# arhix52/Strelka

Measured on AMD Instinct MI355X. Metric: Mray/s, higher is better.
Workload: dtype f32; 1 GPU; kitchen stand-in (SURVEY 8d C3): 1724134 unique triangles, 2022 instances of 153 meshes, 4 rect + 1 distant light, 60/25/10/5 % diffuse/glossy/metal/glass; resolution=1920x1080, bounces=4, spp=64, tile=32, world_size=1, parallelism=single GPU, rays_per_frame=839862650

## Files before the change

strelka_amd/csrc/skh_kernels.h:

```cpp
#pragma once
#include "skh_bvh.h"
#include "skh_env.h"
#include "skh_emit.h"
#include "skh_blend.h"

namespace skh
{

struct DevInstance
{
    float w2o[12];
    int rootRef;
    uint32_t mask;
    uint32_t type;
    uint32_t pad;
};
struct HostInstance
{
    float o2w[12];
    uint32_t type, geom, material, light;
};

#define SKH_WORLD_CURVES 2
#define SKH_SEG_STRIDE 8
// ... 444 lines not shown
        atomicAdd(&stats->rayTicksAfterDry[A], rayTicks);
        atomicAdd(&stats->waveTicksAfterDry[A], now - dryAt);
    }
#endif
    if (COUNT)
    {
        const uint32_t a = wave_sum(tc.nodes), b = wave_sum(tc.prims), c2 = wave_sum(tc.segs), d2 = wave_sum(tc.insts);
#ifdef SKH_LANE_PROFILE
        cy[5] = __builtin_readcyclecounter() - cyStart;
        if (lane == 0)
        {
            atomicAdd(&stats->cyc[ANY_HIT ? 1 : 0][6], cy[5]);
            atomicAdd(&stats->cyc[ANY_HIT ? 1 : 0][7], __builtin_amdgcn_s_memrealtime() - rtStart);
        }
        for (int k = 0; k < 7; ++k)
        {
            uint32_t hi = wave_max((uint32_t)(cy[k] >> 8));
            if (lane == 0)
                atomicAdd(&stats->cyc[ANY_HIT ? 1 : 0][k == 6 ? 8 : k], (unsigned long long)hi << 8);
        }
#endif
        if (lane == 0)
        {
            atomicAdd(&stats->nodes[ANY_HIT ? 1 : 0], (unsigned long long)a);
            atomicAdd(&stats->prims[ANY_HIT ? 1 : 0], (unsigned long long)b);
            atomicAdd(&stats->segs[ANY_HIT ? 1 : 0], (unsigned long long)c2);
            atomicAdd(&stats->insts[ANY_HIT ? 1 : 0], (unsigned long long)d2);
#ifdef SKH_LANE_PROFILE
            for (int k = 0; k < 10; ++k)
                atomicAdd(&stats->wave[ANY_HIT ? 1 : 0][k], (unsigned long long)wv[k]);
#endif
        }
    }
#undef SKH_LP
}

__global__ void k_hair_consts(const Material* __restrict__ mats, uint32_t n, HairConst* __restrict__ out)
{
    const uint32_t i = blockIdx.x * blockDim.x + threadIdx.x;
    if (i < n)
        out[i] = hair_const(mats[i]);
}

SKH_DI bool slot_to_pixel(const FrameP& fp, const uint32_t* __restrict__ tileXY, uint32_t slot, uint32_t& px, uint32_t& py)
{
    const uint32_t tile = slot >> (2 * fp.tileShift);
    const uint32_t m = slot & ((1u << (2 * fp.tileShift)) - 1u);
    px = tileXY[2 * tile] + compact1by1(m);
    py = tileXY[2 * tile + 1] + compact1by1(m >> 1);
    return px < fp.width && py < fp.height;
}

#define SKH_COMPACT_MAX_WAVES 8
SKH_DI uint32_t block_compact(bool emit, uint32_t* counter, uint32_t* s_wave )
{
    const uint32_t lane = threadIdx.x & 63u, wave = threadIdx.x >> 6, nw = blockDim.x >> 6;
    const unsigned long long m = __ballot(emit);
    if (lane == 0)
        s_wave[wave] = (uint32_t)__popcll(m);
    __syncthreads();
    if (threadIdx.x == 0)
    {
        uint32_t tot = 0;
        for (uint32_t w = 0; w < nw; ++w)
        {
            const uint32_t cnt = s_wave[w];
            s_wave[w] = tot;
            tot += cnt;
        }
        s_wave[SKH_COMPACT_MAX_WAVES] = tot ? atomicAdd(counter, tot) : 0u;
    }
    __syncthreads();
    const uint32_t r = s_wave[SKH_COMPACT_MAX_WAVES] + s_wave[wave] + rank_below(m);
    __syncthreads();
    return r;
}
SKH_DI void block_compact2(bool emitA, uint32_t* counterA, bool emitB, uint32_t* counterB, uint32_t* s_wave2, uint32_t& ia, uint32_t& ib)
{
    const uint32_t lane = threadIdx.x & 63u, wave = threadIdx.x >> 6, nw = blockDim.x >> 6;
    const unsigned long long ma = __ballot(emitA), mb = __ballot(emitB);
    uint32_t* sa = s_wave2;
    uint32_t* sb = s_wave2 + SKH_COMPACT_MAX_WAVES + 1;
    if (lane == 0)
    {
        sa[wave] = (uint32_t)__popcll(ma);
        sb[wave] = (uint32_t)__popcll(mb);
    }
    __syncthreads();
    if (threadIdx.x == 0 || threadIdx.x == 64)
    {
        uint32_t* sw = threadIdx.x == 0 ? sa : sb;
        uint32_t tot = 0;
        for (uint32_t w = 0; w < nw; ++w)
        {
            const uint32_t cnt = sw[w];
            sw[w] = tot;
            tot += cnt;
        }
        sw[SKH_COMPACT_MAX_WAVES] = tot ? atomicAdd(threadIdx.x == 0 ? counterA : counterB, tot) : 0u;
    }
    if (nw == 1 && threadIdx.x == 0)
    {
        uint32_t tot = sb[0];
        sb[0] = 0;
        sb[SKH_COMPACT_MAX_WAVES] = tot ? atomicAdd(counterB, tot) : 0u;
    }
    __syncthreads();
    ia = sa[SKH_COMPACT_MAX_WAVES] + sa[wave] + rank_below(ma);
    ib = sb[SKH_COMPACT_MAX_WAVES] + sb[wave] + rank_below(mb);
}

__global__ void __launch_bounds__(512) k_raygen(FrameP fp, const uint32_t* __restrict__ tileXY, uint32_t sampleOffset, RayQ rq,
                                               uint32_t* __restrict__ counter, PathS ps, const uint32_t* __restrict__ qBase,
                                               const uint32_t* __restrict__ subStride, uint32_t blocksPerSub, uint32_t validPerSub,
                                               uint32_t launchCell, uint32_t perWave)
{
    __shared__ uint32_t s_wave[SKH_COMPACT_MAX_WAVES + 1];
    const uint32_t span = launchCell * fp.batch, lc = blockIdx.x / span, inSpan = blockIdx.x - lc * span;
    const uint32_t nb = min(launchCell, blocksPerSub - lc * launchCell);
    const uint32_t sub = inSpan / nb, bi = lc * launchCell + (inSpan - sub * nb);
    const uint32_t slot = bi * blockDim.x + threadIdx.x;
    const uint32_t path = sub * fp.numSlots + slot;
    uint32_t px = 0, py = 0;
    const bool active = sub < fp.batch && slot < fp.numSlots && slot_to_pixel(fp, tileXY, slot, px, py);
    v3 o = mk3(0.0f), d = mk3(0.0f);
    if (active)
    {
// ... 206 lines not shown
}
SKH_DI v3 emit_sample_texel(const MtexP& m, const DevScene& sc, uint32_t instance, uint32_t prim, float ux, float uy)
{
    const HostInstance* __restrict__ hi = sc.instances + instance;
    const uint32_t mid0 = hi->material == 0xffffffffu ? 0u : hi->material, mid = mid0 < sc.numMaterials ? mid0 : 0u;
    const MtexEntry e = mtex_entry(m, mid);
    if (!mtex_valid(e.emission_texture, sc.numTextures))
        return mk3(1.0f);
    const float4* __restrict__ tp = sc.shadeTris + 6 * (size_t)(hi->light + prim);
    const float4 t3 = tp[3], t4 = tp[4];
    float u0, v0, u1, v1, u2, v2;
    unpack_uv(__float_as_uint(t3.w), u0, v0);
    unpack_uv(__float_as_uint(t4.x), u1, v1);
    unpack_uv(__float_as_uint(t4.y), u2, v2);
    const float su = sqrtf(ux);
    const float b0 = 1.0f - su, b1 = su * (1.0f - uy), b2 = su * uy;
    return mtex_emission_texel(tex_lookup_rgba8(sc.texels, sc.texDesc[e.emission_texture - 1u], (u0 * b0 + u1 * b1) + u2 * b2, (v0 * b0 + v1 * b1) + v2 * b2),
                               e.emission_channel);
}
__global__ void __launch_bounds__(256) k_material_probe(MtexP mt, const Material* __restrict__ materials, uint32_t numMaterials, const float4* __restrict__ Le,
                                                        const uint32_t* __restrict__ texels, const uint4* __restrict__ texDesc, uint32_t numTextures,
                                                        const uint32_t* __restrict__ material, const float* __restrict__ uv, uint32_t n, float* __restrict__ out)
{
    const uint32_t i = blockIdx.x * blockDim.x + threadIdx.x;
    if (i >= n)
        return;
    const uint32_t mid0 = material[i] == 0xffffffffu ? 0u : material[i], mid = mid0 < numMaterials ? mid0 : 0u;
    Material mat = materials[mid];
    const float4 l = Le[mid];
    v3 le = mk3(l.x, l.y, l.z);
    resolve_material(texels, texDesc, numTextures, mat, mtex_entry(mt, mid), le, uv[2 * (size_t)i], uv[2 * (size_t)i + 1]);
    float* o = out + 8 * (size_t)i;
    o[0] = mat.base_color[0], o[1] = mat.base_color[1], o[2] = mat.base_color[2], o[3] = mat.roughness, o[4] = mat.metallic;
    o[5] = le.x, o[6] = le.y, o[7] = le.z;
}
__global__ void __launch_bounds__(256) k_emit_probe_mtex(EmitP em, MtexP mt, DevScene sc, const float* __restrict__ in, uint32_t n, uint32_t* __restrict__ out)
{
    const uint32_t i = blockIdx.x * blockDim.x + threadIdx.x;
    if (i >= n)
        return;
    const float* q = in + 6 * (size_t)i;
    const EmitSample s = emit_sample(em, q[0], q[1], q[2], mk3(q[3], q[4], q[5]));
    const v3 Le = s.Le * emit_sample_texel(mt, sc, s.instance, s.prim, q[1], q[2]);
    uint32_t* o = out + 13 * (size_t)i;
    o[0] = __float_as_uint(s.point.x), o[1] = __float_as_uint(s.point.y), o[2] = __float_as_uint(s.point.z);
    o[3] = __float_as_uint(s.normal.x), o[4] = __float_as_uint(s.normal.y), o[5] = __float_as_uint(s.normal.z);
    o[6] = __float_as_uint(Le.x), o[7] = __float_as_uint(Le.y), o[8] = __float_as_uint(Le.z);
    o[9] = __float_as_uint(s.pdf), o[10] = __float_as_uint(s.dist), o[11] = s.instance, o[12] = s.prim;
}

#ifndef SKH_SHADE_WAVES
#define SKH_SHADE_WAVES(HAIR) ((HAIR) ? 4 : 5)
#endif
#define SKH_SHADE_ATTR(HAIR) __attribute__((amdgpu_waves_per_eu(SKH_SHADE_WAVES(HAIR), SKH_SHADE_WAVES(HAIR))))
#ifndef SKH_SHADE_BLOCK
#define SKH_SHADE_BLOCK 256
#endif
template <bool HAIR, bool ENV, bool EMIT, bool MTEX>
__global__ void __launch_bounds__(SKH_SHADE_BLOCK) SKH_SHADE_ATTR(HAIR)
    k_shade(DevScene sc, FrameP fp, uint32_t sampleOffset, uint32_t depth , const uint32_t* __restrict__ tileXY, RayQ rq,
            const uint32_t* __restrict__ countPtr, HitQ hq, PathS ps, RayQ nextQ, uint32_t* __restrict__ nextCount, RayQ shadowQ,
            float4* __restrict__ contrib, uint32_t* __restrict__ shadowCount, EnvP env, EmitP emit, MtexP mtex)
{
    constexpr bool LSHAPE = false;
    const LshapeP lsh = { nullptr };
#include "skh_shade_body.inc"
}
template <bool HAIR, bool ENV, bool EMIT, bool MTEX>
__global__ void __launch_bounds__(SKH_SHADE_BLOCK) SKH_SHADE_ATTR(HAIR)
    k_shade_lshape(DevScene sc, FrameP fp, uint32_t sampleOffset, uint32_t depth , const uint32_t* __restrict__ tileXY, RayQ rq,
                   const uint32_t* __restrict__ countPtr, HitQ hq, PathS ps, RayQ nextQ, uint32_t* __restrict__ nextCount, RayQ shadowQ,
                   float4* __restrict__ contrib, uint32_t* __restrict__ shadowCount, EnvP env, EmitP emit, MtexP mtex, LshapeP lsh)
{
    constexpr bool LSHAPE = true;
#include "skh_shade_body.inc"
}

__global__ void __launch_bounds__(256) k_lshape_probe(const Light* __restrict__ lights, uint32_t numLights, LshapeP lsh, uint32_t rectMethod, uint32_t kind,
                                                      const uint32_t* __restrict__ in, uint32_t n, float* __restrict__ out)
{
    const uint32_t i = blockIdx.x * blockDim.x + threadIdx.x;
    if (i >= n)
        return;
    const uint32_t* q = in + (kind == 0u ? 6u : 7u) * (size_t)i;
    const uint32_t lid = q[0];
    float* o = out + (kind == 0u ? 13u : 2u) * (size_t)i;
    if (lid >= numLights)
    {
        for (uint32_t k = 0; k < (kind == 0u ? 13u : 2u); ++k)
            o[k] = 0.0f;
        return;
    }
    const Light light = lights[lid];
    Lshape lse;
    lse.flags = 0u, lse.cosOuter = lse.cosInner = lse.focus = 0.0f, lse.axis = mk3(0.0f);
    if (lsh.table)
        lse = lshape_fetch(lsh, lid);
    const bool sampledDisc = light.type == 1 && (lse.flags & SKH_LSHAPE_SAMPLE_DISC) != 0u;
    if (kind == 0u)
    {
        const float ux = __uint_as_float(q[1]), uy = __uint_as_float(q[2]);
        const v3 P = mk3(__uint_as_float(q[3]), __uint_as_float(q[4]), __uint_as_float(q[5]));
        LightSample d;
        d.pointOnLight = mk3(0.0f), d.pdf = 0.0f, d.normal = mk3(0.0f), d.area = 0.0f, d.L = mk3(0.0f), d.distToLight = 0.0f;
        switch (light.type)
        {
        case 0:
            d = rectMethod == 0u ? sample_rect_light_uniform(light, ux, uy, P) : sample_rect_light(light, ux, uy, P);
            break;
        case 1:
            if (sampledDisc)
                d = sample_disc_light(light, ux, uy, P);
            break;
        case 2:
            d = sample_sphere_light(light, ux, uy, P);
            break;
        case 3:
            d = sample_distant_light(light, ux, uy);
            break;
        default:
            break;
        }
// ... 667 lines not shown
```

strelka_amd/csrc/skh_shade_body.inc:

```
    const uint32_t numPick = (ENV ? sc.numLights + (env.nee ? 1u : 0u) : sc.numLights) + (EMIT ? (emit.nee ? 1u : 0u) : 0u);
    __shared__ uint32_t s_wave[2 * (SKH_COMPACT_MAX_WAVES + 1)];
    __shared__ uint32_t s_sobol[SKH_SOBOL_LUT_WORDS];
#if SKH_MATERIALS_LDS
    __shared__ float4 s_mat[SKH_MATERIALS_LDS * 4];
#endif
    const uint32_t shard = blockIdx.x & (SKH_SHARDS - 1u), lb = blockIdx.x / SKH_SHARDS;
    const uint32_t n = countPtr[shard * SKH_COUNT_STRIDE];
    if (lb * blockDim.x >= n)
        return;
    const uint32_t il = lb * blockDim.x + threadIdx.x;
    const uint32_t i = shard * rq.region + il;
#ifdef SKH_LANE_PROFILE
    unsigned long long spc[8] = { 0, 0, 0, 0, 0, 0, 0, 0 }, spT = __builtin_readcyclecounter();
#define SKH_SP(k)                                                    \
    {                                                                \
        const unsigned long long t_ = __builtin_readcyclecounter();  \
        spc[k] += t_ - spT;                                          \
        spT = t_;                                                    \
    }
#else
#define SKH_SP(k)
#endif
    bool valid = il < n;
    uint32_t pid = 0;
    v3 rayO = mk3(0.0f), rayD = mk3(0.0f);
    float4 hr0 = make_float4(0.0f, 0.0f, 0.0f, 0.0f), hr1 = hr0;
    {
        constexpr int passes = ((SKH_SOBOL_LUT_WORDS / 4) + SKH_SHADE_BLOCK - 1) / SKH_SHADE_BLOCK;
        uint4 lut[passes];
#pragma unroll
        for (int k = 0; k < passes; ++k)
            if ((k + 1) * SKH_SHADE_BLOCK <= SKH_SOBOL_LUT_WORDS / 4 || threadIdx.x + k * SKH_SHADE_BLOCK < SKH_SOBOL_LUT_WORDS / 4)
                lut[k] = reinterpret_cast<const uint4*>(g_sobol_lut)[threadIdx.x + k * SKH_SHADE_BLOCK];
            else
                lut[k] = make_uint4(0u, 0u, 0u, 0u);
#if SKH_MATERIALS_LDS
        float4 mrow = make_float4(0.0f, 0.0f, 0.0f, 0.0f);
        static_assert(SKH_MATERIALS_LDS * 4 <= SKH_SHADE_BLOCK, "one float4 of the material table per thread");
        if (threadIdx.x < SKH_MATERIALS_LDS * 4 && threadIdx.x < sc.numMaterials * 4u)
            mrow = reinterpret_cast<const float4*>(sc.materials)[threadIdx.x];
#endif
#pragma unroll
        for (int k = 0; k < passes; ++k)
            if ((k + 1) * SKH_SHADE_BLOCK <= SKH_SOBOL_LUT_WORDS / 4 || threadIdx.x + k * SKH_SHADE_BLOCK < SKH_SOBOL_LUT_WORDS / 4)
                reinterpret_cast<uint4*>(s_sobol)[threadIdx.x + k * SKH_SHADE_BLOCK] = lut[k];
#if SKH_MATERIALS_LDS
        if (threadIdx.x < SKH_MATERIALS_LDS * 4)
            s_mat[threadIdx.x] = mrow;
#endif
    }
    __syncthreads();
    bool emitNext = false, emitShadow = false;
    v3 nextO = mk3(0.0f), nextD = mk3(0.0f), shO = mk3(0.0f), shD = mk3(0.0f), shC = mk3(0.0f);
    float shTmax = 0.0f;
    if (valid)
    {
        pid = rq.ids()[i];
        rayO = mk3(rq.plane(0)[i], rq.plane(1)[i], rq.plane(2)[i]);
        rayD = mk3(rq.plane(3)[i], rq.plane(4)[i], rq.plane(5)[i]);
        if (hq.primBits != 0u)
        {
            hr0 = *hq.rec16(i);
            const uint32_t w = __float_as_uint(hr0.w);
            hr1.x = __uint_as_float(w == 0xffffffffu ? w : w >> hq.primBits);
            hr1.y = __uint_as_float(w == 0xffffffffu ? w : ((w & ((1u << hq.primBits) - 1u)) | (hq.direct ? SKH_PRIM_DIRECT : 0u)));
        }
        else
            hr0 = hq.rec(i)[0], hr1 = hq.rec(i)[1];
        const float ht = hr0.x, hu = hr0.y, hv = hr0.z;
        const uint32_t hinst = __float_as_uint(hr1.x), hprim = __float_as_uint(hr1.y);
        float* P = ps.base;
        const size_t S = ps.stride;
        v3 throughput = depth == 0u ? mk3(1.0f) : mk3(P[pid], P[pid + S], P[pid + 2 * S]);
        v3 radiance = mk3(0.0f);
        bool radianceDirty = false;
#define SKH_RADIANCE_LOAD() radiance = mk3(ps.rad()[pid]), radianceDirty = true
        float lastBsdfPdf = depth == 0u ? 0.0f : P[pid + 6 * S];
        uint32_t flags = depth == 0u ? 0u : reinterpret_cast<uint32_t*>(P)[pid + 7 * S];
        bool inside = (flags & PF_INSIDE) != 0;
        bool specularBounce = (flags & PF_SPECULAR) != 0;
        uint32_t firstEvent = (flags >> PF_EVENT_SHIFT) & 3u;
        uint32_t px, py;
        const uint32_t sub = pid / fp.numSlots;
        slot_to_pixel(fp, tileXY, pid - sub * fp.numSlots, px, py);
        Sampler smp = init_sampler(px, py, fp.subframeIndex + sampleOffset + sub, fp.sppTotal, 52u);
        smp.depth = depth;
        uint32_t prdDepth = depth;
        v3 origin = rayO, dir = rayD;

        if (hinst == 0xffffffffu)
        {
            if constexpr (ENV)
            {
                const EnvEval ee = env_eval(env, rayD);
                SKH_RADIANCE_LOAD();
                if (depth == 0 || specularBounce || !env.nee)
                    radiance = radiance + throughput * ee.Le;
                else
                {
                    const float lightPdf = ee.pdf / (float)numPick;
                    const float misWeight = mis_weight_balance(lastBsdfPdf, lightPdf);
                    radiance = radiance + throughput * ee.Le * misWeight;
                }
            }
            else
            {
                const v3 bg = throughput * mk3(0.0f);
                if (!(bg.x == 0.0f && bg.y == 0.0f && bg.z == 0.0f))
                {
                    SKH_RADIANCE_LOAD();
                    radiance = radiance + bg;
                }
            }
            throughput = mk3(0.0f);
            prdDepth = fp.maxDepth;
        }
        else
        {
            SKH_SP(0)
            const HostInstance hi = sc.instances[hinst];
            const float* w2o = sc.inst[hinst].w2o;
            const bool directTv = (hprim & SKH_PRIM_DIRECT) != 0u;
            float4 tv[3], tx[2];
            const bool txWanted = HAIR || sc.numTextures != 0u;
            tx[0] = tx[1] = make_float4(0.0f, 0.0f, 0.0f, 0.0f);
            {
                const uint32_t recIdx = directTv ? (hprim & ~SKH_PRIM_DIRECT) : 0u;
                const float4* tp = sc.shadeTris + 6 * (size_t)(hq.primBits ? min(recIdx, hq.recClamp) : recIdx);
#pragma unroll
                for (int k = 0; k < 3; ++k)
                    tv[k] = tp[k];
                if (txWanted)
                    tx[0] = tp[3], tx[1] = tp[4];
            }
            asm volatile("" ::"v"(hi.type), "v"(hi.material), "v"(hi.light));
            if (hi.type == 1)
            {
                const uint32_t lidx = hi.light < sc.numLights ? hi.light : 0u;
                const Light& l = sc.lights[lidx];
                const v3 hitPoint = rayO + ht * rayD;
                if constexpr (LSHAPE)
                {
                    const Lshape lse = lshape_fetch(lsh, lidx);
                    const bool sampledDisc = l.type == 1 && (lse.flags & SKH_LSHAPE_SAMPLE_DISC) != 0u;
                    const v3 lightNormal = sampledDisc ? normalize(mk3(l.normal)) : calc_light_normal(l, hitPoint);
                    if (-dot(rayD, lightNormal) > 0.0f)
                    {
                        const v3 Li = mk3(l.color) * lshape_cone(lse, -rayD);
                        SKH_RADIANCE_LOAD();
                        if (depth == 0 || specularBounce)
                            radiance = radiance + throughput * Li * -dot(rayD, lightNormal);
                        else
                        {
                            const float lightPdf = (sampledDisc ? disc_light_pdf(l, hitPoint, rayO) : get_light_pdf(l, hitPoint, rayO)) / (float)numPick;
                            const float misWeight = mis_weight_balance(lastBsdfPdf, lightPdf);
                            radiance = radiance + throughput * Li * -dot(rayD, lightNormal) * misWeight;
                        }
                    }
                }
                else
                {
                    const v3 lightNormal = calc_light_normal(l, hitPoint);
                    if (-dot(rayD, lightNormal) > 0.0f)
                    {
                        SKH_RADIANCE_LOAD();
                        if (depth == 0 || specularBounce)
                            radiance = radiance + throughput * mk3(l.color) * -dot(rayD, lightNormal);
                        else
                        {
                            const float lightPdf = get_light_pdf(l, hitPoint, rayO) / (float)numPick;
                            const float misWeight = mis_weight_balance(lastBsdfPdf, lightPdf);
                            radiance = radiance + throughput * mk3(l.color) * -dot(rayD, lightNormal) * misWeight;
                        }
                    }
                }
                throughput = mk3(0.0f);
            }
            else
            {
                const uint32_t mid = hi.material == 0xffffffffu ? 0u : hi.material;
                float4 matLe = make_float4(0.0f, 0.0f, 0.0f, 0.0f);
                if constexpr (EMIT)
                    matLe = emit.Le[mid < emit.numMaterials ? mid : 0u];
                MtexEntry mte;
                if constexpr (MTEX)
                    mte = mtex_entry(mtex, mid < sc.numMaterials ? mid : 0u);
#if SKH_MATERIALS_LDS
                const uint32_t midc = mid < sc.numMaterials ? mid : 0u;
                Material mat;
                if (midc < (uint32_t)SKH_MATERIALS_LDS)
                {
                    const float4 m0 = s_mat[4 * midc], m1 = s_mat[4 * midc + 1], m2 = s_mat[4 * midc + 2], m3 = s_mat[4 * midc + 3];
                    mat.type = __float_as_uint(m0.x), mat.base_color[0] = m0.y, mat.base_color[1] = m0.z, mat.base_color[2] = m0.w;
                    mat.roughness = m1.x, mat.metallic = m1.y, mat.specular = m1.z, mat.ior = m1.w;
                    mat.base_color_texture = __float_as_uint(m2.x), mat.normal_texture = __float_as_uint(m2.y);
                    mat.reserved[0] = m2.z, mat.reserved[1] = m2.w, mat.reserved[2] = m3.x, mat.reserved[3] = m3.y, mat.reserved[4] = m3.z, mat.reserved[5] = m3.w;
                }
                else
                    mat = sc.materials[midc];
#else
                Material mat = sc.materials[mid < sc.numMaterials ? mid : 0u];
#endif
                if (!directTv && hi.type != 2)
                {
                    const float4* tp = sc.shadeTris + 6 * (size_t)(hi.light + hprim);
#pragma unroll
                    for (int k = 0; k < 3; ++k)
                        tv[k] = tp[k];
                    if (txWanted)
                        tx[0] = tp[3], tx[1] = tp[4];
                }
                asm volatile("" ::"v"(mat.type), "v"(tv[0].x), "v"(tv[1].x), "v"(tv[2].x));
                const bool useBase = mat.base_color_texture != 0u && mat.base_color_texture <= sc.numTextures;
                const bool useNormal = mat.normal_texture != 0u && mat.normal_texture <= sc.numTextures;
                bool mtexWanted = false;
                if constexpr (MTEX)
                    mtexWanted = mtex_wanted(mat, mte, sc.numTextures, matLe.w > 0.0f);
                const bool textured = hi.type != 2 && (useBase || useNormal || mtexWanted);
                SurfaceTex st;
                v3 stT = mk3(0.0f);
                const bool hairOnMesh = HAIR && mat.type == 3u && hi.type != 2;
                SurfaceHit sh = hi.type == 2 ? fill_curve(sc, hi, w2o, hprim & ~SKH_PRIM_DIRECT , hu, ht, rayO, rayD, inside, HAIR ? &stT : nullptr) :
                                               fill_triangle(hi, w2o, tv, tx, hu, hv, inside, (textured || hairOnMesh) ? &st : nullptr);
                if (hairOnMesh)
                    stT = st.tangent_u;
                if (textured)
                {
                    if constexpr (MTEX)
                    {
                        v3 Le = mk3(matLe.x, matLe.y, matLe.z);
                        resolve_material(sc.texels, sc.texDesc, sc.numTextures, mat, mte, Le, st.u, st.v);
                        matLe.x = Le.x, matLe.y = Le.y, matLe.z = Le.z;
                    }
                    else if (useBase)
                    {
                        const v4 c = tex_lookup_rgba8(sc.texels, sc.texDesc[mat.base_color_texture - 1u], st.u, st.v);
                        mat.base_color[0] = c.x, mat.base_color[1] = c.y, mat.base_color[2] = c.z;
                    }
                    if (useNormal)
                    {
                        const v4 c = tex_lookup_rgba8(sc.texels, sc.texDesc[mat.normal_texture - 1u], st.u, st.v);
                        const v3 ts = mk3(c.x * 2.0f - 1.0f, c.y * 2.0f - 1.0f, c.z * 2.0f - 1.0f);
                        sh.normal = normalize((st.tangent_u * ts.x + st.tangent_v * ts.y) + sh.normal * ts.z);
                    }
                }
                if (fp.debug == 1)
                    radiance = (sh.normal + mk3(1.0f)) * 0.5f, radianceDirty = true;
                else
                {
                    if constexpr (EMIT)
                    {
                        if (hi.type == 0u && matLe.w > 0.0f)
                        {
                            const v3 ne = inside ? -sh.geom_normal : sh.geom_normal;
                            if (-dot(rayD, ne) > 0.0f)
                            {
                                const v3 Le = mk3(matLe.x, matLe.y, matLe.z);
                                SKH_RADIANCE_LOAD();
                                if (depth == 0 || specularBounce || !emit.nee)
                                    radiance = radiance + throughput * Le;
                                else
                                {
                                    const float lightPdf = emit_pdf(ne, matLe.w * emit.invSumW, sh.position, rayO) / (float)numPick;
                                    const float misWeight = mis_weight_balance(lastBsdfPdf, lightPdf);
                                    radiance = radiance + throughput * Le * misWeight;
                                }
                            }
                        }
                    }
                    const float xi0 = sampler_random_lut(smp, DIM_BSDF0, s_sobol), xi1 = sampler_random_lut(smp, DIM_BSDF1, s_sobol),
                                xi2 = sampler_random_lut(smp, DIM_BSDF2, s_sobol);
                    const float xi3 = HAIR ? sampler_random_lut(smp, DIM_BSDF3, s_sobol) : 0.0f;
                    const v3 k1 = -rayD;
                    BsdfSample bs;
                    SKH_SP(1)
                    v3 toLight = mk3(0.0f);
                    float lightPdf = 0.0f;
                    v3 lrad = mk3(0.0f);
                    bool wantShadow = false;
                    float distToLight = 0.0f;
                    auto sampleLight = [&]() {
                        if (numPick > 0)
                        {
                            const float u = sampler_random_lut(smp, DIM_LIGHT_ID, s_sobol);
                            const uint32_t lightId = (uint32_t)((float)numPick * u);
                            const float lightSelectionPdf = 1.0f / (float)numPick;
                            if constexpr (EMIT)
                            {
                                if (emit.nee && lightId + 1u >= numPick)
                                {
                                    const float uSel = fminf(fmaxf((float)numPick * u - (float)(numPick - 1u), 0.0f), 0.99999994f);
                                    const float ux = sampler_random_lut(smp, DIM_LIGHT_X, s_sobol), uy = sampler_random_lut(smp, DIM_LIGHT_Y, s_sobol);
                                    const EmitSample es = emit_sample(emit, uSel, ux, uy, sh.position);
                                    toLight = es.L;
                                    if (dot(sh.normal, es.L) > 0.0f && -dot(es.L, es.normal) > 0.0f && es.pdf > 0.0f)
                                    {
                                        wantShadow = true;
                                        distToLight = es.dist * (1.0f - SKH_EMIT_SHADOW_MARGIN);
                                        lightPdf = es.pdf;
                                        lrad = es.Le;
                                        if constexpr (MTEX)
                                            lrad = lrad * emit_sample_texel(mtex, sc, es.instance, es.prim, ux, uy);
                                    }
                                    lightPdf *= lightSelectionPdf;
                                    return;
                                }
                            }
                            if constexpr (ENV)
                            {
                                if (lightId >= sc.numLights)
                                {
                                    const float ux = sampler_random_lut(smp, DIM_LIGHT_X, s_sobol), uy = sampler_random_lut(smp, DIM_LIGHT_Y, s_sobol);
// ... 26 lines not shown
                            d.area = 0.0f;
                            d.L = mk3(0.0f);
                            d.distToLight = 0.0f;
                            switch (light.type)
                            {
                            case 0:
                                d = fp.rectMethod == 0 ? sample_rect_light_uniform(light, ux, uy, sh.position) :
                                                         sample_rect_light(light, ux, uy, sh.position);
                                break;
                            case 1:
                                if constexpr (LSHAPE)
                                {
                                    if (lse.flags & SKH_LSHAPE_SAMPLE_DISC)
                                        d = sample_disc_light(light, ux, uy, sh.position);
                                }
                                break;
                            case 2:
                                d = sample_sphere_light(light, ux, uy, sh.position);
                                break;
                            case 3:
                                d = sample_distant_light(light, ux, uy);
                                break;
                            default:
                                break;
                            }
                            toLight = d.L;
                            v3 Li = mk3(light.color);
                            if constexpr (LSHAPE)
                                Li = Li * lshape_cone(lse, -d.L);
                            if (dot(sh.normal, d.L) > 0.0f && -dot(d.L, d.normal) > 0.0f && all3(Li))
                            {
                                wantShadow = true;
                                distToLight = d.distToLight;
                                lightPdf = d.pdf;
                                lrad = 1.0f * Li * saturatef(dot(sh.normal, d.L));
                            }
                            lightPdf *= lightSelectionPdf;
                        }
                    };
                    const bool hairHit = HAIR && mat.type == 3u;
                    BsdfEval evHair;
                    bool evHairDone = false;
                    if (hairHit)
                    {
                        sampleLight();
                        evHairDone = !(isnan3(lrad) || isnan(lightPdf)) && (((dot(toLight, sh.normal) > 0.0f) != inside) && lightPdf != 0.0f);
                        hair_sample_and_evaluate(mat, sh.normal, sh.geom_normal, stT, k1, xi0, xi1, xi2, xi3, sc.hairConst + (mid < sc.numMaterials ? mid : 0u), bs, evHairDone, toLight, evHair);
                    }
                    else
                        bsdf_sample<HAIR>(mat, sh.normal, sh.geom_normal, stT, k1, xi0, xi1, xi2, xi3, inside, bs, HAIR ? sc.hairConst + (mid < sc.numMaterials ? mid : 0u) : nullptr);
                    SKH_SP(2)
                    if (bs.event_type == EV_ABSORB)
                    {
                        if (depth == 0)
                            firstEvent = 1;
                        throughput = mk3(0.0f);
                    }
                    else
                    {
                        specularBounce = (bs.event_type & EV_SPECULAR) != 0;
                        if (depth == 0)
                        {
                            if (bs.event_type & EV_DIFFUSE)
                                firstEvent = 2;
                            if (bs.event_type & EV_GLOSSY)
                                firstEvent = 3;
                        }
                        bool errorOut = false;
                        if (bs.event_type & (EV_DIFFUSE | EV_GLOSSY))
                        {
                            if (!hairHit)
                                sampleLight();
                            if (isnan3(lrad) || isnan(lightPdf))
                            {
                                radiance = mk3(10000.0f, 0.0f, 0.0f), radianceDirty = true;
                                throughput = mk3(0.0f);
                                errorOut = true;
                            }
                            else
                            {
                                const bool isNextEventValid = ((dot(toLight, sh.normal) > 0.0f) != inside) && lightPdf != 0.0f;
                                if (isNextEventValid)
                                {
                                    BsdfEval ev;
                                    SKH_SP(3)
                                    if (hairHit)
                                        ev = evHair;
                                    else
                                        bsdf_evaluate<HAIR>(mat, sh.normal, sh.geom_normal, stT, k1, toLight, inside, ev, HAIR ? sc.hairConst + (mid < sc.numMaterials ? mid : 0u) : nullptr);
                                    SKH_SP(4)
                                    if (isnan3(ev.bsdf_diffuse) || isnan3(ev.bsdf_glossy))
                                    {
                                        radiance = mk3(10000.0f, 0.0f, 0.0f), radianceDirty = true;
                                        throughput = mk3(0.0f);
                                        errorOut = true;
                                    }
                                    else if (ev.pdf > 0.0f && wantShadow)
                                    {
                                        const v3 radianceOverPdf = lrad / lightPdf;
                                        const float misWeight = mis_weight_balance(lightPdf, ev.pdf);
                                        shC = throughput * radianceOverPdf * misWeight * (ev.bsdf_diffuse + ev.bsdf_glossy);
                                        shO = offset_ray(sh.position, sh.geom_normal);
                                        shD = toLight;
                                        shTmax = distToLight;
                                        emitShadow = true;
                                    }
                                }
                            }
                        }
                        if (!errorOut)
                        {
                            if (bs.event_type & EV_TRANSMISSION)
                            {
                                inside = !inside;
                                origin = offset_ray(sh.position, -sh.geom_normal);
                            }
                            else
                                origin = offset_ray(sh.position, sh.geom_normal);
                            lastBsdfPdf = specularBounce ? 1.0f : bs.pdf;
                            dir = bs.k2;
                            throughput = throughput * bs.bsdf_over_pdf;
                        }
                    }
                }
            }
        }
        SKH_SP(5)
        bool alive = true;
        if (prdDepth > 3)
        {
            const float p = fmaxf(throughput.x, fmaxf(throughput.y, throughput.z));
            if (sampler_random_lut(smp, DIM_RR, s_sobol) > p)
                alive = false;
            else
                throughput = throughput * (1.0f / (p + 1e-5f));
        }
        if (alive && dot(throughput, throughput) < 1e-5f)
            alive = false;
        if (alive)
        {
            ++prdDepth;
            if (fp.debug == 1)
                alive = false;
        }
        if (alive && prdDepth >= fp.maxDepth)
            alive = false;
        emitNext = alive;
        nextO = origin;
        nextD = dir;
        P[pid] = throughput.x;
        P[pid + S] = throughput.y;
        P[pid + 2 * S] = throughput.z;
        if (radianceDirty)
        {
            ps.rad()[pid] = make_float4(radiance.x, radiance.y, radiance.z, 0.0f);
        }
#undef SKH_RADIANCE_LOAD
        P[pid + 6 * S] = lastBsdfPdf;
        reinterpret_cast<uint32_t*>(P)[pid + 7 * S] =
            (inside ? PF_INSIDE : 0u) | (specularBounce ? PF_SPECULAR : 0u) | (firstEvent << PF_EVENT_SHIFT);
    }
    SKH_SP(6)
    uint32_t ni, si;
    block_compact2(emitNext, nextCount + shard * SKH_COUNT_STRIDE, emitShadow, shadowCount + shard * SKH_COUNT_STRIDE, s_wave, ni, si);
    ni += shard * nextQ.region;
    si += shard * shadowQ.region;
    if (emitNext)
    {
        nextQ.plane(0)[ni] = nextO.x;
        nextQ.plane(1)[ni] = nextO.y;
        nextQ.plane(2)[ni] = nextO.z;
        nextQ.plane(3)[ni] = nextD.x;
        nextQ.plane(4)[ni] = nextD.y;
        nextQ.plane(5)[ni] = nextD.z;
        nextQ.ids()[ni] = pid;
    }
    if (emitShadow)
    {
        shadowQ.plane(0)[si] = shO.x;
        shadowQ.plane(1)[si] = shO.y;
        shadowQ.plane(2)[si] = shO.z;
        shadowQ.plane(3)[si] = shD.x;
        shadowQ.plane(4)[si] = shD.y;
        shadowQ.plane(5)[si] = shD.z;
        shadowQ.plane(7)[si] = shTmax;
        contrib[si] = make_float4(shC.x, shC.y, shC.z, __uint_as_float(pid));
    }
#ifdef SKH_LANE_PROFILE
    SKH_SP(7)
    for (int k = 0; k < 8; ++k)
    {
        const uint32_t hi32 = wave_max((uint32_t)(spc[k] >> 4));
        if ((threadIdx.x & 63u) == 0)
            atomicAdd(&sc.profile->shade[k], (unsigned long long)hi32 << 4);
    }
#endif
#undef SKH_SP
```

strelka_amd/csrc/strelka_hip.hip:

```cpp
#include "../../include/strelka_hip.h"
#include "skh_kernels.h"

#include <dlfcn.h>
typedef struct ncclComm* ncclComm_t;
typedef struct
{
    char internal[128];
} ncclUniqueId;
typedef enum
{
    ncclSuccess = 0
} ncclResult_t;
typedef enum
{
    ncclFloat = 7
} ncclDataType_t;

#include <algorithm>
#include <chrono>
#include <cmath>
#include <cstdio>
#include <cstring>
#include <mutex>
#include <string>
#include <vector>

using namespace skh;

static_assert(sizeof(skh_vertex) == 32 && sizeof(skh_instance) == 64 && sizeof(skh_light) == 112, "ABI layout");
static_assert(sizeof(skh_material) == 64 && sizeof(skh_frame_params) == 176 && sizeof(skh_ray) == 32, "ABI layout");
static_assert(sizeof(skh_hit) == 20 && sizeof(Light) == 112 && sizeof(Material) == 64 && sizeof(HostInstance) == 64, "layout");

#include "skh_host.h"
#include "skh_aov.h"
#include "skh_denoise.h"
#include "skh_temporal.h"
#include "skh_variance.h"
#include "skh_motion.h"
#include "skh_rectify.h"

static void init_sobol_table(uint32_t tab[5][32])
{
    for (int i = 0; i < 32; ++i)
        tab[0][i] = 1u << (31 - i);
    const int S[4] = { 1, 2, 3, 3 };
    const uint32_t A[4] = { 0, 1, 1, 2 };
    const uint32_t M[4][3] = { { 1, 0, 0 }, { 1, 3, 0 }, { 1, 3, 1 }, { 1, 1, 1 } };
    for (int d = 0; d < 4; ++d)
    {
        uint32_t* v = tab[d + 1];
        const int s = S[d];
        for (int i = 0; i < s; ++i)
            v[i] = M[d][i] << (31 - i);
        for (int i = s; i < 32; ++i)
        {
            uint32_t x = v[i - s] ^ (v[i - s] >> s);
            for (int k = 1; k < s; ++k)
                if ((A[d] >> (s - 1 - k)) & 1u)
                    x ^= v[i - k];
            v[i] = x;
        }
    }
}



static void spec_drop(skh_context* c, bool keepLast = false, bool keepAdaptive = false)
{
    skh_context::Speculation& sp = c->spec;
    if (!keepLast && !keepAdaptive)
        c->adapt.ready = false;
    if (sp.nextInFlight)
    {
        unsigned long long after[2] = { 0, 0 };
        (void)hipStreamSynchronize(c->dev.stream);
        if (hipMemcpy(after, c->timing.dStats.p, sizeof(after), hipMemcpyDeviceToHost) == hipSuccess)
        {
            c->spec.discardedRadiance += after[0] - sp.statsMark[0];
            c->spec.discardedShadow += after[1] - sp.statsMark[1];
        }
        c->spec.discardedSubframes += sp.nextCount;
        sp.nextInFlight = false;
    }
    if (sp.valid && sp.consumed < sp.count && sp.count > 0)
    {
        const uint32_t left = sp.count - sp.consumed;
        c->spec.discardedRadiance += sp.passRadiance * left / sp.count;
        c->spec.discardedShadow += sp.passShadow * left / sp.count;
        c->spec.discardedSubframes += left;
    }
    sp.valid = false;
    sp.buf = 0;
// ... 1715 lines not shown
    hipStream_t st;
    const uint32_t* tiles;
    PathS ps;
    RayQ rq[2], shq, cutQ[2], cutSQ[2];
    HitQ hq, cutH, cutSH0, cutSH1;
    uint32_t *counts, *fetch, *cutWords;
    uint32_t QW, NP, rounds, cutBounceWords;
    bool smallPass, useOverlap, split, cutOn;
    BlendP blp;
};

static FrameP frame_params(const skh_context* c, const skh_frame_params* p, const RenderPlan& plan)
{
    FrameP fp;
    memcpy(fp.viewToWorld, p->view_to_world, sizeof(fp.viewToWorld));
    memcpy(fp.clipToView, p->clip_to_view, sizeof(fp.clipToView));
    fp.subframeIndex = p->subframe_index;
    fp.samplesThisLaunch = p->samples_this_launch;
    fp.sppTotal = p->spp_total;
    fp.maxDepth = p->max_depth;
    fp.rectMethod = p->rect_light_sampling_method;
    memcpy(fp.exposure, p->exposure, sizeof(fp.exposure));
    fp.enableAccumulation = p->enable_accumulation;
    fp.debug = p->debug;
    fp.shadowTmin = p->shadow_ray_tmin;
    fp.materialTmin = p->material_ray_tmin;
    frame_geometry(c, fp);
    fp.batch = plan.batch;
    fp.finalFirst = std::min(plan.finalFirst, plan.batch);
    fp.finalCount = std::min(plan.finalCount, plan.batch - fp.finalFirst);
    return fp;
}

static void fill_queue_constants(skh_context* c, const RenderPass& rp)
{
    const uint32_t NQ = rp.shq.stride;
    uint32_t bits[2];
    memcpy(&bits[0], &rp.fp.materialTmin, 4);
    memcpy(&bits[1], &rp.fp.shadowTmin, 4);
    if (c->frame.queueConstFilled && bits[0] == c->frame.queueConstBits[0] && bits[1] == c->frame.queueConstBits[1])
        return;
    const uint32_t fb = (uint32_t)c->dev.numCUs * 8u;
    for (int k = 0; k < 2; ++k)
    {
        k_fill_f32<<<fb, 256, 0, rp.st>>>(rp.rq[k].base + (size_t)6 * NQ, NQ, rp.fp.materialTmin);
        k_fill_f32<<<fb, 256, 0, rp.st>>>(rp.rq[k].base + (size_t)7 * NQ, NQ, 1e16f);
    }
    k_fill_f32<<<fb, 256, 0, rp.st>>>(rp.shq.base + (size_t)6 * NQ, NQ, rp.fp.shadowTmin);
    c->frame.queueConstFilled = true;
    c->frame.queueConstBits[0] = bits[0];
    c->frame.queueConstBits[1] = bits[1];
}

#define SKH_SHADE_BUILDS(K)                                                                                                                      \
    {                                                                                                                                            \
        K<false, false, false, false>, K<false, false, false, true>, K<false, false, true, false>, K<false, false, true, true>,                  \
        K<false, true, false, false>, K<false, true, false, true>, K<false, true, true, false>, K<false, true, true, true>,                      \
        K<true, false, false, false>, K<true, false, false, true>, K<true, false, true, false>, K<true, false, true, true>,                      \
        K<true, true, false, false>, K<true, true, false, true>, K<true, true, true, false>, K<true, true, true, true>                           \
    }
static const decltype(&k_shade<false, false, false, false>) kShadeKernels[16] = SKH_SHADE_BUILDS(k_shade);
static const decltype(&k_shade_lshape<false, false, false, false>) kShadeLshapeKernels[16] = SKH_SHADE_BUILDS(k_shade_lshape);
#undef SKH_SHADE_BUILDS

static void launch_shade(skh_context* c, const RenderPass& rp, uint32_t s, uint32_t b)
{
    const uint32_t perShard = (((rp.NP + SKH_SHARDS - 1u) / SKH_SHARDS) + 63u) & ~63u;
    const dim3 sg(SKH_SHARDS * ((perShard + SKH_SHADE_BLOCK - 1) / SKH_SHADE_BLOCK));
    const uint32_t build = (c->scene.hasHairMaterial ? 8u : 0u) | (c->env.w ? 4u : 0u) | (rp.emitp.count ? 2u : 0u) | (rp.mtexp.count ? 1u : 0u), QW = rp.QW;
    uint32_t* counts = rp.counts;
    if (rp.lshp.table)
        kShadeLshapeKernels[build]<<<sg, SKH_SHADE_BLOCK, 0, rp.st>>>(rp.sc, rp.fp, s, b, rp.tiles, rp.rq[b & 1], counts + 2 * b * QW, rp.hq, rp.ps, rp.rq[(b + 1) & 1],
                                                                      counts + 2 * (b + 1) * QW, rp.shq, c->frame.dContrib.as<float4>(), counts + (2 * b + 1) * QW, rp.envp,
                                                                      rp.emitp, rp.mtexp, rp.lshp);
    else
        kShadeKernels[build]<<<sg, SKH_SHADE_BLOCK, 0, rp.st>>>(rp.sc, rp.fp, s, b, rp.tiles, rp.rq[b & 1], counts + 2 * b * QW, rp.hq, rp.ps, rp.rq[(b + 1) & 1],
                                                                counts + 2 * (b + 1) * QW, rp.shq, c->frame.dContrib.as<float4>(), counts + (2 * b + 1) * QW, rp.envp, rp.emitp,
                                                                rp.mtexp);
}

static void render_bounce(skh_context* c, const RenderPass& rp, uint32_t s, uint32_t b)
{
    hipStream_t st = rp.st;
    const bool smallGrids = rp.useOverlap && rp.smallPass;
    BlendP blp = rp.blp;
    blp.depth = b;
    uint32_t* words = rp.cutOn ? rp.cutWords + (size_t)b * rp.cutBounceWords : nullptr;
    TraceLaunch t;
    t.ps = rp.ps, t.split = rp.split, t.any = false;
    {
        SpanGuard g(c, KC_TRACE_CLOSEST);
        t.rq = rp.rq[b & 1], t.counts = rp.counts + 2 * b * rp.QW, t.fetch = rp.fetch + 16 * b * SKH_FETCH_STRIDE, t.hq = rp.hq, t.contrib = nullptr, t.stream = st;
        t.smallGrid = smallGrids ? ((b == 0 && c->opt.smallWavesFirst) ? c->opt.smallWavesFirst : c->opt.smallWavesClosest ? c->opt.smallWavesClosest : (c->accel.nSegs ? 16u : 20u)) * (uint32_t)c->dev.numCUs : 0u;
        const CutRounds cr{ { rp.cutQ[0], rp.cutQ[1] }, rp.hq, rp.cutH, nullptr, words, rp.NP, blp };
        trace_step(c, rp.sc, t, false, rp.cutOn ? &cr : nullptr);
    }
    if (rp.useOverlap && b > 0)
        (void)hipStreamWaitEvent(st, c->dev.evShadow, 0);
    {
        SpanGuard g(c, KC_SHADE);
        launch_shade(c, rp, s, b);
    }
    hipStream_t sst = rp.useOverlap ? c->dev.stream2 : st;
    if (rp.useOverlap)
    {
        (void)hipEventRecord(c->dev.evShade, st);
        (void)hipStreamWaitEvent(sst, c->dev.evShade, 0);
    }
    {
        SpanGuard g(c, KC_TRACE_SHADOW, sst);
        t.rq = rp.shq, t.counts = rp.counts + (2 * b + 1) * rp.QW, t.fetch = rp.fetch + (16 * b + 8) * SKH_FETCH_STRIDE, t.hq = HitQ{ nullptr, 0 }, t.contrib = c->frame.dContrib.as<float4>(), t.stream = sst;
        t.smallGrid = smallGrids ? ((b + 1 == rp.rounds && (c->opt.smallWavesLast || (!c->opt.smallWavesShadow && !c->accel.nSegs))) ? (c->opt.smallWavesLast ? c->opt.smallWavesLast : 20u) : c->opt.smallWavesShadow ? c->opt.smallWavesShadow : (c->accel.nSegs ? 16u : 12u)) * (uint32_t)c->dev.numCUs : 0u;
        const CutRounds cr{ { rp.cutSQ[0], rp.cutSQ[1] }, rp.cutSH0, rp.cutSH1, nullptr, rp.cutOn ? words + c->opt.cutoutRounds * SKH_CUT_WORDS : nullptr, rp.NP, blp };
        trace_step(c, rp.sc, t, true, rp.cutOn ? &cr : nullptr);
    }
    if (rp.useOverlap)
        (void)hipEventRecord(c->dev.evShadow, sst);
}

static void render_accumulate(skh_context* c, const RenderPass& rp, const RenderPlan& plan, bool oneSampleDirect, void* d_image)
{
    if (!plan.finalize)
        return;
    const uint32_t gridSlots = (c->frame.numSlots + 255) / 256;
    const bool fromPaths = plan.batch > 1 || oneSampleDirect;
    hipStream_t fs = plan.finStream ? plan.finStream : rp.st;
    {
        SpanGuard g(c, KC_ACCUM, fs);
        if (fromPaths)
// ... 1748 lines not shown
```

Measured before the change: 6512 Mray/s.

## Specialize shade kernel by bounce position to skip state writes on last bounce

Adds a POS template parameter to the shade kernels and builds separate first, middle and last bounce variants, picked at launch from the bounce index. The last-bounce variant skips Russian roulette, next-ray generation, path-state stores and the next-queue compaction, uses a single-queue compaction without the trailing barrier, and may run at higher occupancy (6 waves per EU) when no hair, emissive, texture or lshape features are present. The first-bounce variant folds the depth==0 checks into constants. The cost is three times as many kernel instantiations and the risk that the MIDDLE/stateInit handling diverges from the original depth semantics.

```diff
diff --git a/strelka_amd/csrc/skh_kernels.h b/strelka_amd/csrc/skh_kernels.h
--- a/strelka_amd/csrc/skh_kernels.h
+++ b/strelka_amd/csrc/skh_kernels.h
@@ -520,7 +520,7 @@
 }
 
 #define SKH_COMPACT_MAX_WAVES 8
-SKH_DI uint32_t block_compact(bool emit, uint32_t* counter, uint32_t* s_wave )
+SKH_DI uint32_t block_compact(bool emit, uint32_t* counter, uint32_t* s_wave , bool reuse = true )
 {
     const uint32_t lane = threadIdx.x & 63u, wave = threadIdx.x >> 6, nw = blockDim.x >> 6;
     const unsigned long long m = __ballot(emit);
@@ -540,7 +540,8 @@
     }
     __syncthreads();
     const uint32_t r = s_wave[SKH_COMPACT_MAX_WAVES] + s_wave[wave] + rank_below(m);
-    __syncthreads();
+    if (reuse)
+        __syncthreads();
     return r;
 }
 SKH_DI void block_compact2(bool emitA, uint32_t* counterA, bool emitB, uint32_t* counterB, uint32_t* s_wave2, uint32_t& ia, uint32_t& ib)
@@ -853,12 +854,27 @@
 #ifndef SKH_SHADE_WAVES
 #define SKH_SHADE_WAVES(HAIR) ((HAIR) ? 4 : 5)
 #endif
-#define SKH_SHADE_ATTR(HAIR) __attribute__((amdgpu_waves_per_eu(SKH_SHADE_WAVES(HAIR), SKH_SHADE_WAVES(HAIR))))
+enum
+{
+    SHADE_ANY = 0,
+    SHADE_FIRST,
+    SHADE_MIDDLE,
+    SHADE_LAST
+};
+#ifndef SKH_SHADE_POSITIONS
+#define SKH_SHADE_POSITIONS 1
+#endif
+#ifndef SKH_SHADE_WAVES_LAST
+#define SKH_SHADE_WAVES_LAST(HAIR, EMIT, MTEX, LSHAPE) ((HAIR) || (EMIT) || (MTEX) || (LSHAPE) ? SKH_SHADE_WAVES(HAIR) : 6)
+#endif
+#define SKH_SHADE_WAVES_AT(HAIR, EMIT, MTEX, LSHAPE, POS) ((POS) == SHADE_LAST ? SKH_SHADE_WAVES_LAST(HAIR, EMIT, MTEX, LSHAPE) : SKH_SHADE_WAVES(HAIR))
+#define SKH_SHADE_ATTR(HAIR, EMIT, MTEX, LSHAPE, POS) \
+    __attribute__((amdgpu_waves_per_eu(SKH_SHADE_WAVES_AT(HAIR, EMIT, MTEX, LSHAPE, POS), SKH_SHADE_WAVES_AT(HAIR, EMIT, MTEX, LSHAPE, POS))))
 #ifndef SKH_SHADE_BLOCK
 #define SKH_SHADE_BLOCK 256
 #endif
-template <bool HAIR, bool ENV, bool EMIT, bool MTEX>
-__global__ void __launch_bounds__(SKH_SHADE_BLOCK) SKH_SHADE_ATTR(HAIR)
+template <bool HAIR, bool ENV, bool EMIT, bool MTEX, int POS>
+__global__ void __launch_bounds__(SKH_SHADE_BLOCK) SKH_SHADE_ATTR(HAIR, EMIT, MTEX, false, POS)
     k_shade(DevScene sc, FrameP fp, uint32_t sampleOffset, uint32_t depth , const uint32_t* __restrict__ tileXY, RayQ rq,
             const uint32_t* __restrict__ countPtr, HitQ hq, PathS ps, RayQ nextQ, uint32_t* __restrict__ nextCount, RayQ shadowQ,
             float4* __restrict__ contrib, uint32_t* __restrict__ shadowCount, EnvP env, EmitP emit, MtexP mtex)
@@ -867,8 +883,8 @@
     const LshapeP lsh = { nullptr };
 #include "skh_shade_body.inc"
 }
-template <bool HAIR, bool ENV, bool EMIT, bool MTEX>
-__global__ void __launch_bounds__(SKH_SHADE_BLOCK) SKH_SHADE_ATTR(HAIR)
+template <bool HAIR, bool ENV, bool EMIT, bool MTEX, int POS>
+__global__ void __launch_bounds__(SKH_SHADE_BLOCK) SKH_SHADE_ATTR(HAIR, EMIT, MTEX, true, POS)
     k_shade_lshape(DevScene sc, FrameP fp, uint32_t sampleOffset, uint32_t depth , const uint32_t* __restrict__ tileXY, RayQ rq,
                    const uint32_t* __restrict__ countPtr, HitQ hq, PathS ps, RayQ nextQ, uint32_t* __restrict__ nextCount, RayQ shadowQ,
                    float4* __restrict__ contrib, uint32_t* __restrict__ shadowCount, EnvP env, EmitP emit, MtexP mtex, LshapeP lsh)
diff --git a/strelka_amd/csrc/skh_shade_body.inc b/strelka_amd/csrc/skh_shade_body.inc
--- a/strelka_amd/csrc/skh_shade_body.inc
+++ b/strelka_amd/csrc/skh_shade_body.inc
@@ -1,3 +1,6 @@
+    constexpr bool kLast = POS == SHADE_LAST;
+    const bool depth0 = POS == SHADE_ANY ? depth == 0u : POS == SHADE_FIRST;
+    const bool stateInit = POS == SHADE_MIDDLE ? depth == 0u : depth0;
     const uint32_t numPick = (ENV ? sc.numLights + (env.nee ? 1u : 0u) : sc.numLights) + (EMIT ? (emit.nee ? 1u : 0u) : 0u);
     __shared__ uint32_t s_wave[2 * (SKH_COMPACT_MAX_WAVES + 1)];
     __shared__ uint32_t s_sobol[SKH_SOBOL_LUT_WORDS];
@@ -71,12 +74,12 @@
         const uint32_t hinst = __float_as_uint(hr1.x), hprim = __float_as_uint(hr1.y);
         float* P = ps.base;
         const size_t S = ps.stride;
-        v3 throughput = depth == 0u ? mk3(1.0f) : mk3(P[pid], P[pid + S], P[pid + 2 * S]);
+        v3 throughput = stateInit ? mk3(1.0f) : mk3(P[pid], P[pid + S], P[pid + 2 * S]);
         v3 radiance = mk3(0.0f);
         bool radianceDirty = false;
 #define SKH_RADIANCE_LOAD() radiance = mk3(ps.rad()[pid]), radianceDirty = true
-        float lastBsdfPdf = depth == 0u ? 0.0f : P[pid + 6 * S];
-        uint32_t flags = depth == 0u ? 0u : reinterpret_cast<uint32_t*>(P)[pid + 7 * S];
+        float lastBsdfPdf = stateInit ? 0.0f : P[pid + 6 * S];
+        uint32_t flags = stateInit ? 0u : reinterpret_cast<uint32_t*>(P)[pid + 7 * S];
         bool inside = (flags & PF_INSIDE) != 0;
         bool specularBounce = (flags & PF_SPECULAR) != 0;
         uint32_t firstEvent = (flags >> PF_EVENT_SHIFT) & 3u;
@@ -84,8 +87,8 @@
         const uint32_t sub = pid / fp.numSlots;
         slot_to_pixel(fp, tileXY, pid - sub * fp.numSlots, px, py);
         Sampler smp = init_sampler(px, py, fp.subframeIndex + sampleOffset + sub, fp.sppTotal, 52u);
-        smp.depth = depth;
-        uint32_t prdDepth = depth;
+        smp.depth = POS == SHADE_FIRST ? 0u : depth;
+        uint32_t prdDepth = smp.depth;
         v3 origin = rayO, dir = rayD;
 
         if (hinst == 0xffffffffu)
@@ -94,7 +97,7 @@
             {
                 const EnvEval ee = env_eval(env, rayD);
                 SKH_RADIANCE_LOAD();
-                if (depth == 0 || specularBounce || !env.nee)
+                if (depth0 || specularBounce || !env.nee)
                     radiance = radiance + throughput * ee.Le;
                 else
                 {
@@ -148,7 +151,7 @@
                     {
                         const v3 Li = mk3(l.color) * lshape_cone(lse, -rayD);
                         SKH_RADIANCE_LOAD();
-                        if (depth == 0 || specularBounce)
+                        if (depth0 || specularBounce)
                             radiance = radiance + throughput * Li * -dot(rayD, lightNormal);
                         else
                         {
@@ -164,7 +167,7 @@
                     if (-dot(rayD, lightNormal) > 0.0f)
                     {
                         SKH_RADIANCE_LOAD();
-                        if (depth == 0 || specularBounce)
+                        if (depth0 || specularBounce)
                             radiance = radiance + throughput * mk3(l.color) * -dot(rayD, lightNormal);
                         else
                         {
@@ -257,7 +260,7 @@
                             {
                                 const v3 Le = mk3(matLe.x, matLe.y, matLe.z);
                                 SKH_RADIANCE_LOAD();
-                                if (depth == 0 || specularBounce || !emit.nee)
+                                if (depth0 || specularBounce || !emit.nee)
                                     radiance = radiance + throughput * Le;
                                 else
                                 {
@@ -390,14 +393,14 @@
                     SKH_SP(2)
                     if (bs.event_type == EV_ABSORB)
                     {
-                        if (depth == 0)
+                        if (depth0)
                             firstEvent = 1;
                         throughput = mk3(0.0f);
                     }
                     else
                     {
                         specularBounce = (bs.event_type & EV_SPECULAR) != 0;
-                        if (depth == 0)
+                        if (depth0)
                         {
                             if (bs.event_type & EV_DIFFUSE)
                                 firstEvent = 2;
@@ -446,7 +449,7 @@
                                 }
                             }
                         }
-                        if (!errorOut)
+                        if (!kLast && !errorOut)
                         {
                             if (bs.event_type & EV_TRANSMISSION)
                             {
@@ -464,46 +467,57 @@
             }
         }
         SKH_SP(5)
-        bool alive = true;
-        if (prdDepth > 3)
+        if constexpr (kLast)
         {
-            const float p = fmaxf(throughput.x, fmaxf(throughput.y, throughput.z));
-            if (sampler_random_lut(smp, DIM_RR, s_sobol) > p)
+            if (radianceDirty)
+                ps.rad()[pid] = make_float4(radiance.x, radiance.y, radiance.z, 0.0f);
+        }
+        else
+        {
+            bool alive = true;
+            if (prdDepth > 3)
+            {
+                const float p = fmaxf(throughput.x, fmaxf(throughput.y, throughput.z));
+                if (sampler_random_lut(smp, DIM_RR, s_sobol) > p)
+                    alive = false;
+                else
+                    throughput = throughput * (1.0f / (p + 1e-5f));
+            }
+            if (alive && dot(throughput, throughput) < 1e-5f)
                 alive = false;
-            else
-                throughput = throughput * (1.0f / (p + 1e-5f));
-        }
-        if (alive && dot(throughput, throughput) < 1e-5f)
-            alive = false;
-        if (alive)
-        {
-            ++prdDepth;
-            if (fp.debug == 1)
+            if (alive)
+            {
+                ++prdDepth;
+                if (fp.debug == 1)
+                    alive = false;
+            }
+            if (alive && prdDepth >= fp.maxDepth)
                 alive = false;
-        }
-        if (alive && prdDepth >= fp.maxDepth)
-            alive = false;
-        emitNext = alive;
-        nextO = origin;
-        nextD = dir;
-        P[pid] = throughput.x;
-        P[pid + S] = throughput.y;
-        P[pid + 2 * S] = throughput.z;
-        if (radianceDirty)
-        {
-            ps.rad()[pid] = make_float4(radiance.x, radiance.y, radiance.z, 0.0f);
+            emitNext = alive;
+            nextO = origin;
+            nextD = dir;
+            P[pid] = throughput.x;
+            P[pid + S] = throughput.y;
+            P[pid + 2 * S] = throughput.z;
+            if (radianceDirty)
+            {
+                ps.rad()[pid] = make_float4(radiance.x, radiance.y, radiance.z, 0.0f);
+            }
+            P[pid + 6 * S] = lastBsdfPdf;
+            reinterpret_cast<uint32_t*>(P)[pid + 7 * S] =
+                (inside ? PF_INSIDE : 0u) | (specularBounce ? PF_SPECULAR : 0u) | (firstEvent << PF_EVENT_SHIFT);
         }
 #undef SKH_RADIANCE_LOAD
-        P[pid + 6 * S] = lastBsdfPdf;
-        reinterpret_cast<uint32_t*>(P)[pid + 7 * S] =
-            (inside ? PF_INSIDE : 0u) | (specularBounce ? PF_SPECULAR : 0u) | (firstEvent << PF_EVENT_SHIFT);
     }
     SKH_SP(6)
-    uint32_t ni, si;
-    block_compact2(emitNext, nextCount + shard * SKH_COUNT_STRIDE, emitShadow, shadowCount + shard * SKH_COUNT_STRIDE, s_wave, ni, si);
+    uint32_t ni = 0, si;
+    if constexpr (kLast)
+        si = block_compact(emitShadow, shadowCount + shard * SKH_COUNT_STRIDE, s_wave, false);
+    else
+        block_compact2(emitNext, nextCount + shard * SKH_COUNT_STRIDE, emitShadow, shadowCount + shard * SKH_COUNT_STRIDE, s_wave, ni, si);
     ni += shard * nextQ.region;
     si += shard * shadowQ.region;
-    if (emitNext)
+    if (!kLast && emitNext)
     {
         nextQ.plane(0)[ni] = nextO.x;
         nextQ.plane(1)[ni] = nextO.y;
diff --git a/strelka_amd/csrc/strelka_hip.hip b/strelka_amd/csrc/strelka_hip.hip
--- a/strelka_amd/csrc/strelka_hip.hip
+++ b/strelka_amd/csrc/strelka_hip.hip
@@ -38,6 +38,7 @@
 #include "skh_variance.h"
 #include "skh_motion.h"
 #include "skh_rectify.h"
+
 
 static void init_sobol_table(uint32_t tab[5][32])
 {
@@ -1859,15 +1860,21 @@
     c->frame.queueConstBits[1] = bits[1];
 }
 
-#define SKH_SHADE_BUILDS(K)                                                                                                                      \
-    {                                                                                                                                            \
-        K<false, false, false, false>, K<false, false, false, true>, K<false, false, true, false>, K<false, false, true, true>,                  \
-        K<false, true, false, false>, K<false, true, false, true>, K<false, true, true, false>, K<false, true, true, true>,                      \
-        K<true, false, false, false>, K<true, false, false, true>, K<true, false, true, false>, K<true, false, true, true>,                      \
-        K<true, true, false, false>, K<true, true, false, true>, K<true, true, true, false>, K<true, true, true, true>                           \
-    }
-static const decltype(&k_shade<false, false, false, false>) kShadeKernels[16] = SKH_SHADE_BUILDS(k_shade);
-static const decltype(&k_shade_lshape<false, false, false, false>) kShadeLshapeKernels[16] = SKH_SHADE_BUILDS(k_shade_lshape);
+#define SKH_SHADE_BUILDS(K, P)                                                                                                                               \
+    {                                                                                                                                                        \
+        K<false, false, false, false, P>, K<false, false, false, true, P>, K<false, false, true, false, P>, K<false, false, true, true, P>,                  \
+        K<false, true, false, false, P>, K<false, true, false, true, P>, K<false, true, true, false, P>, K<false, true, true, true, P>,                      \
+        K<true, false, false, false, P>, K<true, false, false, true, P>, K<true, false, true, false, P>, K<true, false, true, true, P>,                      \
+        K<true, true, false, false, P>, K<true, true, false, true, P>, K<true, true, true, false, P>, K<true, true, true, true, P>                           \
+    }
+#if SKH_SHADE_POSITIONS
+#define SKH_SHADE_TABLE(K) { SKH_SHADE_BUILDS(K, SHADE_FIRST), SKH_SHADE_BUILDS(K, SHADE_MIDDLE), SKH_SHADE_BUILDS(K, SHADE_LAST) }
+#else
+#define SKH_SHADE_TABLE(K) { SKH_SHADE_BUILDS(K, SHADE_ANY), SKH_SHADE_BUILDS(K, SHADE_ANY), SKH_SHADE_BUILDS(K, SHADE_ANY) }
+#endif
+static const decltype(&k_shade<false, false, false, false, SHADE_ANY>) kShadeKernels[3][16] = SKH_SHADE_TABLE(k_shade);
+static const decltype(&k_shade_lshape<false, false, false, false, SHADE_ANY>) kShadeLshapeKernels[3][16] = SKH_SHADE_TABLE(k_shade_lshape);
+#undef SKH_SHADE_TABLE
 #undef SKH_SHADE_BUILDS
 
 static void launch_shade(skh_context* c, const RenderPass& rp, uint32_t s, uint32_t b)
@@ -1876,12 +1883,13 @@
     const dim3 sg(SKH_SHARDS * ((perShard + SKH_SHADE_BLOCK - 1) / SKH_SHADE_BLOCK));
     const uint32_t build = (c->scene.hasHairMaterial ? 8u : 0u) | (c->env.w ? 4u : 0u) | (rp.emitp.count ? 2u : 0u) | (rp.mtexp.count ? 1u : 0u), QW = rp.QW;
     uint32_t* counts = rp.counts;
+    const uint32_t pos = b == 0u ? 0u : b + 1u == rp.rounds ? 2u : 1u;
     if (rp.lshp.table)
-        kShadeLshapeKernels[build]<<<sg, SKH_SHADE_BLOCK, 0, rp.st>>>(rp.sc, rp.fp, s, b, rp.tiles, rp.rq[b & 1], counts + 2 * b * QW, rp.hq, rp.ps, rp.rq[(b + 1) & 1],
+        kShadeLshapeKernels[pos][build]<<<sg, SKH_SHADE_BLOCK, 0, rp.st>>>(rp.sc, rp.fp, s, b, rp.tiles, rp.rq[b & 1], counts + 2 * b * QW, rp.hq, rp.ps, rp.rq[(b + 1) & 1],
                                                                       counts + 2 * (b + 1) * QW, rp.shq, c->frame.dContrib.as<float4>(), counts + (2 * b + 1) * QW, rp.envp,
                                                                       rp.emitp, rp.mtexp, rp.lshp);
     else
-        kShadeKernels[build]<<<sg, SKH_SHADE_BLOCK, 0, rp.st>>>(rp.sc, rp.fp, s, b, rp.tiles, rp.rq[b & 1], counts + 2 * b * QW, rp.hq, rp.ps, rp.rq[(b + 1) & 1],
+        kShadeKernels[pos][build]<<<sg, SKH_SHADE_BLOCK, 0, rp.st>>>(rp.sc, rp.fp, s, b, rp.tiles, rp.rq[b & 1], counts + 2 * b * QW, rp.hq, rp.ps, rp.rq[(b + 1) & 1],
                                                                 counts + 2 * (b + 1) * QW, rp.shq, c->frame.dContrib.as<float4>(), counts + (2 * b + 1) * QW, rp.envp, rp.emitp,
                                                                 rp.mtexp);
 }
```

New measurement: 6591 Mray/s (median of 6 runs). 1.01x the previous value.
